# kungyao/vae-play

Hardware: AMD Instinct MI355X
Metric: images/sec (train step, 128x128 VAE) (higher is better)
Workload: dtype bf16x3; 1 GPU; networks VAE 128x128x3 latent=128 train step (fwd+BCE/KL+bwd+allreduce+Adam), 32 images/GPU, global batch 32; parallelism=dp1, per_gpu_batch=32, global_batch=32, graph=False, precision=bf16x3

## Files before the change

### vae_play_amd/csrc/conv16.hip

```cpp
#define VP_PCFG_LIBRARY 1
#define VP_IGEMM16_M16_ON 1
#include "conv16_impl.h"

namespace vp {

__global__ void split_kernel(const float* __restrict__ x, u16_t* __restrict__ out, size_t n, int fmt, float scale) {
  const size_t n4 = n / 4;
  for (size_t i = (size_t)blockIdx.x * blockDim.x + threadIdx.x; i < n4; i += (size_t)gridDim.x * blockDim.x) {
    const vp_f32x4 v = *reinterpret_cast<const vp_f32x4*>(x + i * 4);
    store_split4(out, n, i * 4, v[0] * scale, v[1] * scale, v[2] * scale, v[3] * scale, fmt);
  }
  if (blockIdx.x == 0 && threadIdx.x < (n & 3)) {
    const size_t i = n4 * 4 + threadIdx.x;
    u16_t h, l;
    split_f32(x[i] * scale, h, l, fmt);
    out[i] = h;
    out[n + i] = l;
  }
}

__global__ void split_pad_kernel(const float* __restrict__ x, u16_t* __restrict__ out, size_t npix, int C, int Cpad) {
  const size_t n = npix * (size_t)Cpad, n4 = n / 4;
  for (size_t i = (size_t)blockIdx.x * blockDim.x + threadIdx.x; i < n4; i += (size_t)gridDim.x * blockDim.x) {
    const size_t e = i * 4, pix = e / Cpad;
    const int c = (int)(e - pix * Cpad);
    const float* src = x + pix * (size_t)C;
    float v[4];
#pragma unroll
    for (int j = 0; j < 4; ++j) v[j] = c + j < C ? src[c + j] : 0.f;
    store_split4(out, n, e, v[0], v[1], v[2], v[3]);
  }
}

template <int MODE, bool SPLIT>
__device__ __forceinline__ void pack_tile(float (*tile)[kTaps + 1], const float* __restrict__ w, void* __restrict__ outv, int Cs,
                                          int Cb, int CsP, int nt, int fixed, int j0, int fmt) {
  const size_t n = (size_t)(MODE == 1 ? CsP : Cs) * Cb * nt;
  const int lim = (MODE == 0 ? Cb : Cs) - j0, lim_out = (MODE == 0 ? Cb : CsP) - j0;
  for (int idx = threadIdx.x; idx < 64 * nt; idx += 256) {
    const int j = idx / nt, t = idx - j * nt;
    if (j < lim) tile[j][t] = w[MODE == 0 ? ((size_t)fixed * Cb + j0 + j) * nt + t : ((size_t)(j0 + j) * Cb + fixed) * nt + t];
  }
  __syncthreads();
  const int inner = MODE == 0 ? Cb : CsP;
  for (int idx = threadIdx.x; idx < 64 * nt; idx += 256) {
    const int t = idx >> 6, j = idx & 63;
    if (j < lim_out) {
      const size_t o = ((size_t)fixed * nt + t) * inner + j0 + j;
      const float v = j < lim ? tile[j][t] : 0.f;
      if constexpr (SPLIT) {
        u16_t h, l;
        split_f32(v, h, l, fmt);
        ((u16_t*)outv)[o] = h;
        ((u16_t*)outv)[n + o] = l;
      } else {
        ((float*)outv)[o] = v;
      }
    }
  }
}

template <int MODE, bool SPLIT>
__global__ void __launch_bounds__(256) pack_w5_tiled_kernel(const float* __restrict__ w, void* __restrict__ outv, int Cs, int Cb,
                                                            int CsP, int nt, int fmt = SPLIT_BF16) {
  __shared__ float tile[64][kTaps + 1];
  pack_tile<MODE, SPLIT>(tile, w, outv, Cs, Cb, CsP, nt, blockIdx.x, blockIdx.y * 64, fmt);
}

template <bool SPLIT>
static int pack_w5_launch(const float* w, void* p0, void* p1, int Cs, int Cb, hipStream_t s, const char* what, int CsP = 0,
                          int nt = kTaps) {
  if (CsP < Cs) CsP = Cs;
  if (p0) hipLaunchKernelGGL((pack_w5_tiled_kernel<0, SPLIT>), dim3(Cs, (Cb + 63) / 64), dim3(256), 0, s, w, p0, Cs, Cb, Cs, nt);
  if (p1) hipLaunchKernelGGL((pack_w5_tiled_kernel<1, SPLIT>), dim3(Cb, (CsP + 63) / 64), dim3(256), 0, s, w, p1, Cs, Cb, CsP, nt);
  return check_launch(what);
}

constexpr int kMaxPackJobs = 32;
struct PackJob { const float* w; void* out; int Cs, Cb, CsP, mode, split, tile_begin; };
struct PackTable { PackJob j[kMaxPackJobs]; int n; };

__global__ void __launch_bounds__(256) pack_w5_batch_kernel(const PackTable tab) {
  __shared__ float tile[64][kTaps + 1];
  int ji = 0;
  for (int k = 1; k < tab.n; ++k)
    if ((int)blockIdx.x >= tab.j[k].tile_begin) ji = k;
  const PackJob& jb = tab.j[ji];
  const int tl = blockIdx.x - jb.tile_begin;
  const int ntile = ((jb.mode == 0 ? jb.Cb : jb.CsP) + 63) / 64;
  const int fixed = tl / ntile, j0 = (tl - fixed * ntile) * 64;
  if (jb.mode == 0) {
    const int fmt = jb.split == 2 ? SPLIT_F16 : SPLIT_BF16;
    if (jb.split) pack_tile<0, true>(tile, jb.w, jb.out, jb.Cs, jb.Cb, jb.CsP, kTaps, fixed, j0, fmt);
    else pack_tile<0, false>(tile, jb.w, jb.out, jb.Cs, jb.Cb, jb.CsP, kTaps, fixed, j0, fmt);
  } else {
    const int fmt = jb.split == 2 ? SPLIT_F16 : SPLIT_BF16;
    if (jb.split) pack_tile<1, true>(tile, jb.w, jb.out, jb.Cs, jb.Cb, jb.CsP, kTaps, fixed, j0, fmt);
    else pack_tile<1, false>(tile, jb.w, jb.out, jb.Cs, jb.Cb, jb.CsP, kTaps, fixed, j0, fmt);
  }
}

int pack_w5_f32_launch(const float* w, float* p0, float* p1, int Cs, int Cb, hipStream_t s, int nt) {
  return pack_w5_launch<false>(w, p0, p1, Cs, Cb, s, "vp_pack_w_f32", 0, nt);
}


static inline int im2col5_gw(int C) { return C == 3 ? 16 : (C == 1 ? 8 : 0); }
static inline int im2col5_kc(int C) { const int g = im2col5_gw(C); return g ? ((5 * g + 31) / 32) * 32 : 0; }

template <int C>
__global__ void __launch_bounds__(256) im2col5s2_split_kernel(const float* __restrict__ x, u16_t* __restrict__ out, int B, int Hb, int Wb,
                                                              int Hs, int Ws, int nchw, int fmt) {
  constexpr int GW = C == 3 ? 16 : 8, KC = ((5 * GW + 31) / 32) * 32, G = KC / 8;
  const size_t npix = (size_t)B * Hs * Ws, n = npix * KC;
  const int row = blockIdx.x, b = row / Hs, hs = row - b * Hs;
  for (int i = threadIdx.x; i < Ws * G; i += blockDim.x) {
    const int ws = i / G, c0 = (i - ws * G) * 8;
    float v[8];
#pragma unroll
    for (int j = 0; j < 8; ++j) {
      const int col = c0 + j, r = col / GW, rem = col - r * GW;
      const int q = rem / C, cin = rem - q * C;
      const int h = 2 * hs - 2 + r, w_ = 2 * ws - 2 + q;
      const bool ok = r < 5 && q < 5 && h >= 0 && h < Hb && w_ >= 0 && w_ < Wb;
      v[j] = ok ? (nchw ? x[(((size_t)b * C + cin) * Hb + h) * Wb + w_] : x[(((size_t)b * Hb + h) * Wb + w_) * C + cin]) : 0.f;
    }
    const size_t o = ((size_t)row * Ws + ws) * KC + c0;
    store_split4(out, n, o, v[0], v[1], v[2], v[3], fmt);
    store_split4(out, n, o + 4, v[4], v[5], v[6], v[7], fmt);
  }
}

template <int C>
__global__ void __launch_bounds__(256) im2col5s2_f32_kernel(const float* __restrict__ x, float* __restrict__ out, int B, int Hb, int Wb,
                                                            int Hs, int Ws, int nchw) {
  constexpr int GW = C == 3 ? 16 : 8, KC = ((5 * GW + 31) / 32) * 32, G = KC / 4;
  const int row = blockIdx.x, b = row / Hs, hs = row - b * Hs;
  for (int i = threadIdx.x; i < Ws * G; i += blockDim.x) {
    const int ws = i / G, c0 = (i - ws * G) * 4;
    vp_f32x4 v;
#pragma unroll
    for (int j = 0; j < 4; ++j) {
      const int col = c0 + j, r = col / GW, rem = col - r * GW;
      const int q = rem / C, cin = rem - q * C;
      const int h = 2 * hs - 2 + r, w_ = 2 * ws - 2 + q;
      const bool ok = r < 5 && q < 5 && h >= 0 && h < Hb && w_ >= 0 && w_ < Wb;
      v[j] = ok ? (nchw ? x[(((size_t)b * C + cin) * Hb + h) * Wb + w_] : x[(((size_t)b * Hb + h) * Wb + w_) * C + cin]) : 0.f;
    }
    *reinterpret_cast<vp_f32x4*>(out + ((size_t)row * Ws + ws) * KC + c0) = v;
  }
}

__global__ void pack_w_im2col5_f32_kernel(const float* __restrict__ w, float* __restrict__ out, int Cout, int C, int GW, int KC) {
  const size_t n = (size_t)Cout * KC;
  for (size_t i = (size_t)blockIdx.x * blockDim.x + threadIdx.x; i < n; i += (size_t)gridDim.x * blockDim.x) {
    const int co = (int)(i / KC), col = (int)(i - (size_t)co * KC);
    const int r = col / GW, rem = col - r * GW, q = rem / C, cin = rem - q * C;
    out[i] = (r < 5 && q < 5) ? w[(((size_t)co * C + cin) * 5 + r) * 5 + q] : 0.f;
  }
}

__global__ void pack_w_im2col5_split_kernel(const float* __restrict__ w, u16_t* __restrict__ out, int Cout, int C, int GW, int KC,
                                            int fmt) {
  const size_t n = (size_t)Cout * KC;
  for (size_t i = (size_t)blockIdx.x * blockDim.x + threadIdx.x; i < n; i += (size_t)gridDim.x * blockDim.x) {
    const int co = (int)(i / KC), col = (int)(i - (size_t)co * KC);
    const int r = col / GW, rem = col - r * GW, q = rem / C, cin = rem - q * C;
    const float v = (r < 5 && q < 5) ? w[(((size_t)co * C + cin) * 5 + r) * 5 + q] : 0.f;
    u16_t h, l;
    split_f32(v, h, l, fmt);
    out[i] = h;
    out[n + i] = l;
  }
}

__global__ void unpack_dw_im2col5_kernel(const float* __restrict__ dwc, float* __restrict__ dw, int Cout, int C, int GW, int KC) {
  const size_t n = (size_t)Cout * C * 25;
  for (size_t i = (size_t)blockIdx.x * blockDim.x + threadIdx.x; i < n; i += (size_t)gridDim.x * blockDim.x) {
    const int q = (int)(i % 5), r = (int)((i / 5) % 5), cin = (int)((i / 25) % C), co = (int)(i / ((size_t)25 * C));
    dw[i] = dwc[(size_t)co * KC + r * GW + q * C + cin];
  }
}

__global__ void __launch_bounds__(256) bn_stats_slab_final_kernel(const float* __restrict__ slab, int G, int tiles_m, int BM, long M, long R,
                                                                  int C, float eps, float momentum, float* __restrict__ mean,
                                                                  float* __restrict__ rstd, float* __restrict__ rm, float* __restrict__ rv) {
  __shared__ double shs[4], shq[4];
  const int c = blockIdx.x;
  const float* pv = slab + ((size_t)0 * C + c) * G;
  const float* sv = slab + ((size_t)1 * C + c) * G;
  const float* qv = slab + ((size_t)2 * C + c) * G;
  const double P = (double)pv[0];
  double S = 0.0, Q = 0.0;
  for (int g = threadIdx.x; g < G; g += 256) {
    const int tile = g % tiles_m;
    const long left = M - (long)tile * BM;
    const double n = (double)(left < BM ? left : BM);
    const double d = (double)pv[g] - P, s = (double)sv[g], q = (double)qv[g];
    S += s + n * d;
    Q += q + 2.0 * d * s + n * d * d;
  }
  S = wave_sum_d(S);
  Q = wave_sum_d(Q);
  if ((threadIdx.x & 63) == 0) { shs[threadIdx.x >> 6] = S; shq[threadIdx.x >> 6] = Q; }
  __syncthreads();
  if (threadIdx.x != 0) return;
  S = (shs[0] + shs[1]) + (shs[2] + shs[3]);
  Q = (shq[0] + shq[1]) + (shq[2] + shq[3]);
  const double ms = S / (double)R;
  double var = Q / (double)R - ms * ms;
  if (var < 0.0) var = 0.0;
  const double m = P + ms;
  mean[c] = (float)m;
  rstd[c] = (float)(1.0 / sqrt(var + (double)eps));
  if (rm) rm[c] = (1.f - momentum) * rm[c] + momentum * (float)m;
  if (rv) {
    const double unb = R > 1 ? var * (double)R / (double)(R - 1) : var;
    rv[c] = (1.f - momentum) * rv[c] + momentum * (float)unb;
  }
}

int stats_finish(const ConvPlan& pl, const StatOut& o, hipStream_t stream, const char* what) {
  hipLaunchKernelGGL(bn_stats_slab_final_kernel, dim3((unsigned)pl.N), dim3(256), 0, stream, (const float*)o.ws, pl.stat_tiles_m * pl.gz,
                     pl.stat_tiles_m, pl.bm, pl.M, pl.stat_R, (int)pl.N, o.eps, o.momentum, o.mean, o.rstd, o.running_mean, o.running_var);
  return check_launch(what);
}

}

using namespace vp;
extern "C" {

static bool split_fmt_ok(int fmt, float scale) { return (fmt == SPLIT_BF16 || fmt == SPLIT_F16) && scale > 0.f; }

int vp_split_fmt_f32(const float* x, void* out_split, size_t n, int fmt, float scale, vp_stream stream) {
  VP_REQUIRE(x && out_split && n > 0, "vp_split_fmt_f32: bad arguments");
  VP_REQUIRE(split_fmt_ok(fmt, scale), "vp_split_fmt_f32: format 0 (bf16 pair) or 1 (fp16 pair), scale > 0");
  hipLaunchKernelGGL(split_kernel, dim3(grid_for(n / 4 + 1, 256)), dim3(256), 0, (hipStream_t)stream, x, (u16_t*)out_split, n, fmt, scale);
  return check_launch("vp_split_fmt_f32");
}

int vp_split_f32(const float* x, void* out_split, size_t n, vp_stream stream) {
  return vp_split_fmt_f32(x, out_split, n, SPLIT_BF16, 1.f, stream);
}

int vp_split_pad_f32(const float* x, void* out_split, size_t npix, int C, int Cpad, vp_stream stream) {
  VP_REQUIRE(x && out_split && npix > 0 && C > 0 && Cpad >= C && Cpad % 8 == 0, "vp_split_pad_f32: Cpad must be a multiple of 8 and >= C");
  hipLaunchKernelGGL(split_pad_kernel, dim3(grid_for(npix * (size_t)Cpad / 4 + 1, 256)), dim3(256), 0, (hipStream_t)stream, x,
                     (u16_t*)out_split, npix, C, Cpad);
  return check_launch("vp_split_pad_f32");
}

int vp_pack_w5_split(const float* w_ref, void* p0_split, void* p1_split, int Csmall, int Cbig, vp_stream stream) {
  VP_REQUIRE(w_ref && (p0_split || p1_split) && Csmall > 0 && Cbig > 0, "vp_pack_w5_split: bad arguments");
  VP_REQUIRE(Csmall <= 65535 && Cbig <= 65535, "vp_pack_w5_split: channel count too large");
  return pack_w5_launch<true>(w_ref, p0_split, p1_split, Csmall, Cbig, (hipStream_t)stream, "vp_pack_w5_split");
}

int vp_pack_w5_batch(const vp_pack_job* jobs, int njobs, vp_stream stream) {
  VP_REQUIRE(jobs && njobs > 0, "vp_pack_w5_batch: bad arguments");
  PackTable tab;
  tab.n = 0;
  int tiles = 0;
  for (int i = 0; i < njobs; ++i) {
    const vp_pack_job& q = jobs[i];
    VP_REQUIRE(q.w && (q.p0 || q.p1) && q.Csmall > 0 && q.Cbig > 0, "vp_pack_w5_batch: job %d: bad arguments", i);
    VP_REQUIRE(q.Csmall <= 65535 && q.Cbig <= 65535, "vp_pack_w5_batch: job %d: channel count too large", i);
    const int CsP = q.Csmall_pad > q.Csmall ? q.Csmall_pad : q.Csmall;
    VP_REQUIRE(CsP == q.Csmall || (q.split && CsP % 8 == 0), "vp_pack_w5_batch: job %d: padding needs split planes and a multiple of 8", i);
    for (int mode = 0; mode < 2; ++mode) {
      void* out = mode == 0 ? q.p0 : q.p1;
      if (!out) continue;
      VP_REQUIRE(tab.n < kMaxPackJobs, "vp_pack_w5_batch: more than %d layouts in one batch", kMaxPackJobs);
      PackJob& j = tab.j[tab.n++];
      j.w = q.w; j.out = out; j.Cs = q.Csmall; j.Cb = q.Cbig; j.CsP = mode == 1 ? CsP : q.Csmall; j.mode = mode;
      j.split = q.split == 2 ? 2 : (q.split ? 1 : 0); j.tile_begin = tiles;
      tiles += mode == 0 ? q.Csmall * ((q.Cbig + 63) / 64) : q.Cbig * ((CsP + 63) / 64);
    }
  }
  hipLaunchKernelGGL(pack_w5_batch_kernel, dim3((unsigned)tiles), dim3(256), 0, (hipStream_t)stream, tab);
  return check_launch("vp_pack_w5_batch");
}

int vp_pack_w5_p1_split_padded(const float* w_ref, void* p1_split, int Csmall, int Cbig, int Csmall_pad, vp_stream stream) {
  VP_REQUIRE(w_ref && p1_split && Csmall > 0 && Cbig > 0 && Csmall_pad >= Csmall && Csmall_pad % 8 == 0,
             "vp_pack_w5_p1_split_padded: bad arguments");
  return pack_w5_launch<true>(w_ref, nullptr, p1_split, Csmall, Cbig, (hipStream_t)stream, "vp_pack_w5_p1_split_padded", Csmall_pad);
}

int vp_conv5_gather_bf16x3(const void* big_split, const void* w_p0_split, const float* bias, float* small_out, int B, int Hs,
                           int Ws, int Cbig, int Csmall, int stride, int act, vp_stream stream) {
  return gather16<0>("vp_conv5_gather_bf16x3", big_split, w_p0_split, bias, small_out, B, Hs, Ws, Hs * stride, Ws * stride, Cbig, Csmall, 5, stride, act, stream);
}

int vp_conv_gather_bf16x3(const void* big_split, const void* w_p0_split, const float* bias, float* small_out, int B, int Hs, int Ws,
                          int Hb, int Wb, int Cbig, int Csmall, int ks, int stride, int act, vp_stream stream) {
  return gather16<0>("vp_conv_gather_bf16x3", big_split, w_p0_split, bias, small_out, B, Hs, Ws, Hb, Wb, Cbig, Csmall, ks, stride, act, stream);
}

int vp_conv5_scatter_bf16x3(const void* small_split, const void* w_p1_split, float* big_out, int B, int Hs, int Ws, int Csmall,
                            int Cbig, int stride, vp_stream stream) {
  return scatter16<0>("vp_conv5_scatter_bf16x3", small_split, w_p1_split, big_out, B, Hs, Ws, Hs * stride, Ws * stride, Csmall, Cbig, 5, stride, stream);
}

int vp_conv_scatter_bf16x3(const void* small_split, const void* w_p1_split, float* big_out, int B, int Hs, int Ws, int Hb, int Wb,
                           int Csmall, int Cbig, int ks, int stride, vp_stream stream) {
  return scatter16<0>("vp_conv_scatter_bf16x3", small_split, w_p1_split, big_out, B, Hs, Ws, Hb, Wb, Csmall, Cbig, ks, stride, stream);
}

int vp_conv_scatter_bias_bf16x3(const void* small_split, const void* w_p1_split, const float* bias, float* big_out, int B, int Hs, int Ws,
                                int Hb, int Wb, int Csmall, int Cbig, int ks, int stride, vp_stream stream) {
  return scatter16<0>("vp_conv_scatter_bias_bf16x3", small_split, w_p1_split, big_out, B, Hs, Ws, Hb, Wb, Csmall, Cbig, ks, stride, stream, 1.f, bias);
}

int vp_pack_w_split(const float* w_ref, void* p0_split, void* p1_split, int Csmall, int Cbig, int ks, vp_stream stream) {
  VP_REQUIRE(w_ref && (p0_split || p1_split) && Csmall > 0 && Cbig > 0, "vp_pack_w_split: bad arguments");
  VP_REQUIRE(ks == 1 || ks == 3 || ks == 4 || ks == 5, "vp_pack_w_split: kernel size must be 1, 3, 4 or 5");
  VP_REQUIRE(Csmall <= 65535 && Cbig <= 65535, "vp_pack_w_split: channel count too large");
  return pack_w5_launch<true>(w_ref, p0_split, p1_split, Csmall, Cbig, (hipStream_t)stream, "vp_pack_w_split", 0, ks * ks);
}

size_t vp_conv5_wgrad_bf16x3_workspace_bytes(int B, int Hs, int Ws, int Cbig, int Csmall, int stride) {
  return vp_conv_wgrad_bf16x3_workspace_bytes(B, Hs, Ws, Hs * stride, Ws * stride, Cbig, Csmall, 5, stride);
}

size_t vp_conv_wgrad_bf16x3_workspace_bytes(int B, int Hs, int Ws, int Hb, int Wb, int Cbig, int Csmall, int ks, int stride) {
  const ConvGeom g = make_geom(B, Hs, Ws, Csmall, Cbig, stride, ks, Hb, Wb);
  return plan_wgrad(g, BF16X3, 0, SIZE_MAX, true, plan_switches()).query_floats * sizeof(float);
}

int vp_conv5_wgrad_bf16x3(const void* big_split, const void* small_split, float* dw_ref, int B, int Hs, int Ws, int Cbig,
                          int Csmall, int stride, void* ws, size_t ws_bytes, vp_stream stream) {
  return wgrad16<0>("vp_conv5_wgrad_bf16x3", big_split, small_split, dw_ref, B, Hs, Ws, Hs * stride, Ws * stride, Cbig, Csmall, 5, stride, ws, ws_bytes, stream);
}

int vp_conv5_wgrad_bf16x3_cus(const void* big_split, const void* small_split, float* dw_ref, int B, int Hs, int Ws, int Cbig,
                              int Csmall, int stride, int max_cus, void* ws, size_t ws_bytes, vp_stream stream) {
  return wgrad16<0>("vp_conv5_wgrad_bf16x3_cus", big_split, small_split, dw_ref, B, Hs, Ws, Hs * stride, Ws * stride, Cbig, Csmall, 5, stride, ws, ws_bytes, stream, 1.f, max_cus);
}

int vp_conv_wgrad_bf16x3(const void* big_split, const void* small_split, float* dw_ref, int B, int Hs, int Ws, int Hb, int Wb, int Cbig,
                         int Csmall, int ks, int stride, void* ws, size_t ws_bytes, vp_stream stream) {
  return wgrad16<0>("vp_conv_wgrad_bf16x3", big_split, small_split, dw_ref, B, Hs, Ws, Hb, Wb, Cbig, Csmall, ks, stride, ws, ws_bytes, stream);
}

size_t vp_conv5_stats_workspace_bytes(int family, int B, int Hs, int Ws, int Cbig, int Csmall, int stride) {
  return plan_stats(family, BF16X3, B, Hs, Ws, Cbig, Csmall, stride, true, plan_switches()).stat_floats * sizeof(float);
}

int vp_conv5_gather_stats_bf16x3(const void* big_split, const void* w_p0_split, float* small_out, int B, int Hs, int Ws, int Cbig,
                                 int Csmall, int stride, float eps, float momentum, float* mean, float* rstd, float* running_mean,
                                 float* running_var, void* ws, size_t ws_bytes, vp_stream stream) {
  return conv5_stats("vp_conv5_gather_stats_bf16x3", "vp_conv5_stats_workspace_bytes", conv_gather<ProbF16, FORMS_ALL, TILES_ALL>, 0, BF16X3, true,
                     big_split, w_p0_split, small_out, B, Hs, Ws, Cbig, Csmall, stride,
                     {eps, momentum, mean, rstd, running_mean, running_var, ws, ws_bytes}, stream);
}

int vp_conv5_scatter_stats_bf16x3(const void* small_split, const void* w_p1_split, float* big_out, int B, int Hs, int Ws, int Csmall,
                                  int Cbig, int stride, float eps, float momentum, float* mean, float* rstd, float* running_mean,
                                  float* running_var, void* ws, size_t ws_bytes, vp_stream stream) {
// ... 73 lines not shown
```

### vae_play_amd/csrc/gemm.hip

```cpp
#include "common.h"
#include "igemm.h"

namespace vp {

__global__ void gemm_reduce_kernel(const float* __restrict__ slab, float* __restrict__ C, const float* __restrict__ bias,
                                   int M, int N, int ldc, int nsplit) {
  const size_t per = (size_t)M * N;
  for (size_t i = (size_t)blockIdx.x * blockDim.x + threadIdx.x; i < per; i += (size_t)gridDim.x * blockDim.x) {
    const int n = (int)(i % N);
    const size_t m = i / N;
    float s = bias ? bias[n] : 0.f;
    for (int sp = 0; sp < nsplit; ++sp) s += slab[(size_t)sp * per + i];
    C[m * ldc + n] = s;
  }
}

__global__ void __launch_bounds__(256) gemm_reduce_deep_kernel(const float* __restrict__ slab, float* __restrict__ C,
                                                               const float* __restrict__ bias, int M, int N, int ldc, int nsplit) {
  __shared__ float red[4][64];
  const size_t per = (size_t)M * N;
  const size_t i = (size_t)blockIdx.x * 64 + (threadIdx.x & 63);
  const int sl = threadIdx.x >> 6;
  float s0 = 0.f, s1 = 0.f, s2 = 0.f, s3 = 0.f;
  if (i < per) {
// ... 3 lines not shown
      s1 += slab[(size_t)(sp + 4) * per + i];
      s2 += slab[(size_t)(sp + 8) * per + i];
      s3 += slab[(size_t)(sp + 12) * per + i];
    }
    for (; sp < nsplit; sp += 4) s0 += slab[(size_t)sp * per + i];
  }
  red[sl][threadIdx.x & 63] = (s0 + s1) + (s2 + s3);
  __syncthreads();
  if (sl == 0 && i < per) {
    const int n = (int)(i % N);
    const size_t m = i / N;
    const float v = (red[0][threadIdx.x] + red[1][threadIdx.x]) + (red[2][threadIdx.x] + red[3][threadIdx.x]);
    C[m * ldc + n] = v + (bias ? bias[n] : 0.f);
  }
}

__global__ void colsum_partial_kernel(const float* __restrict__ x, float* __restrict__ partial, int R, int C, int rows_per_chunk) {
  const int chunk = blockIdx.x;
  const int r0 = chunk * rows_per_chunk;
  const int r1 = min(R, r0 + rows_per_chunk);
  for (int c = threadIdx.y; c < C; c += blockDim.y) {
    float s = 0.f;
    for (int r = r0 + threadIdx.x; r < r1; r += blockDim.x) s += x[(size_t)r * C + c];
    s = wave_sum(s);
    if (threadIdx.x == 0) partial[(size_t)chunk * C + c] = s;
  }
}

__global__ void __launch_bounds__(256) colsum_rows4_kernel(const float* __restrict__ x, float* __restrict__ partial, int R, int C,
                                                           int rows_per_chunk) {
  __shared__ vp_f32x4 sh[256];
  const int q = C / 4, rpp = 256 / q;
  const int rl = threadIdx.x / q, c4 = threadIdx.x - rl * q;
  const int r0 = blockIdx.x * rows_per_chunk, r1 = min(R, r0 + rows_per_chunk);
  vp_f32x4 s = {0.f, 0.f, 0.f, 0.f};
  if (rl < rpp) {
    int r = r0 + rl;
    for (; r + 3 * rpp < r1; r += 4 * rpp) {
      const vp_f32x4 a = *reinterpret_cast<const vp_f32x4*>(x + (size_t)r * C + 4 * c4);
      const vp_f32x4 b = *reinterpret_cast<const vp_f32x4*>(x + (size_t)(r + rpp) * C + 4 * c4);
      const vp_f32x4 c = *reinterpret_cast<const vp_f32x4*>(x + (size_t)(r + 2 * rpp) * C + 4 * c4);
      const vp_f32x4 d = *reinterpret_cast<const vp_f32x4*>(x + (size_t)(r + 3 * rpp) * C + 4 * c4);
#pragma unroll
      for (int j = 0; j < 4; ++j) s[j] += (a[j] + b[j]) + (c[j] + d[j]);
    }
    for (; r < r1; r += rpp) {
      const vp_f32x4 a = *reinterpret_cast<const vp_f32x4*>(x + (size_t)r * C + 4 * c4);
#pragma unroll
      for (int j = 0; j < 4; ++j) s[j] += a[j];
    }
  }
  sh[threadIdx.x] = s;
  __syncthreads();
  if (threadIdx.x < q) {
    vp_f32x4 t = sh[threadIdx.x];
    for (int k = 1; k < rpp; ++k) {
      const vp_f32x4 u = sh[k * q + threadIdx.x];
#pragma unroll
      for (int j = 0; j < 4; ++j) t[j] += u[j];
    }
    *reinterpret_cast<vp_f32x4*>(partial + (size_t)blockIdx.x * C + 4 * threadIdx.x) = t;
  }
}

__global__ void __launch_bounds__(256) colsum_wide_kernel(const float* __restrict__ x, float* __restrict__ partial, int R, int C,
                                                          int rows_per_chunk) {
  const int c = blockIdx.x * 256 + threadIdx.x;
  if (c >= C) return;
  const int r0 = blockIdx.y * rows_per_chunk, r1 = min(R, r0 + rows_per_chunk);
  float s = 0.f;
  for (int r = r0; r < r1; ++r) s += x[(size_t)r * C + c];
  partial[(size_t)blockIdx.y * C + c] = s;
}

__global__ void colsum_final_kernel(const float* __restrict__ partial, float* __restrict__ out, int C, int nchunk) {
  const int c = blockIdx.x;
  double s = 0.0;
  for (int k = threadIdx.x; k < nchunk; k += 64) s += (double)partial[(size_t)k * C + c];
  s = wave_sum_d(s);
  if (threadIdx.x == 0) out[c] = (float)s;
}

constexpr int SK_KT = 64;

template <int TM>
__global__ void __launch_bounds__(256) skinny_mk_kernel(const float* __restrict__ A, long sam, const float* __restrict__ Bm, long sbn,
                                                        float* __restrict__ C, int ldc, const float* __restrict__ bias, int M, int N,
                                                        int K, int nsplit, int kps) {
  __shared__ __attribute__((aligned(16))) float xs[2][32 * TM][SK_KT + 4];
  const int tid = threadIdx.x, lane = tid & 63, wave = tid >> 6;
  const int li = lane & 31, lh = lane >> 5;
  const int n = blockIdx.x * 128 + wave * 32 + li;
  const float* wrow = Bm + (size_t)(n < N ? n : 0) * sbn;
  const int k_begin = blockIdx.y * kps;
  const int k_end = min(K, k_begin + kps);
  const int nk = (k_end - k_begin) / SK_KT;
  const int xrow = tid >> 3, xc = tid & 7;
  const float* arow[TM];
  bool xok[TM];
#pragma unroll
  for (int b = 0; b < TM; ++b) {
    xok[b] = xrow + 32 * b < M;
    arow[b] = A + (size_t)(xok[b] ? xrow + 32 * b : 0) * sam;
  }
  vp_f32x4 xr[TM][2], w[8], wn[8];
  f32x16 acc[TM];
#pragma unroll
  for (int b = 0; b < TM; ++b)
#pragma unroll
    for (int r = 0; r < 16; ++r) acc[b][r] = 0.f;
  auto load_tile = [&](int kb) {
#pragma unroll
    for (int b = 0; b < TM; ++b) {
      xr[b][0] = xok[b] ? ld4(arow[b] + kb + xc * 4) : zero4();
      xr[b][1] = xok[b] ? ld4(arow[b] + kb + 32 + xc * 4) : zero4();
    }
#pragma unroll
    for (int i = 0; i < 8; ++i) wn[i] = ld4(wrow + kb + lh * 32 + i * 4);
  };
  auto write_x = [&](int buf) {
#pragma unroll
    for (int b = 0; b < TM; ++b) {
      *reinterpret_cast<vp_f32x4*>(&xs[buf][xrow + 32 * b][xc * 4]) = xr[b][0];
      *reinterpret_cast<vp_f32x4*>(&xs[buf][xrow + 32 * b][32 + xc * 4]) = xr[b][1];
    }
  };
  if (nk > 0) {
    load_tile(k_begin);
    write_x(0);
    __syncthreads();
  }
  for (int t = 0; t < nk; ++t) {
    const bool more = t + 1 < nk;
#pragma unroll
    for (int i = 0; i < 8; ++i) w[i] = wn[i];
    if (more) load_tile(k_begin + (t + 1) * SK_KT);
    const int cur = t & 1;
#pragma unroll
    for (int i = 0; i < 8; ++i) {
      vp_f32x4 x4[TM];
#pragma unroll
      for (int b = 0; b < TM; ++b) x4[b] = *reinterpret_cast<const vp_f32x4*>(&xs[cur][li + 32 * b][lh * 32 + i * 4]);
#pragma unroll
      for (int j = 0; j < 4; ++j)
#pragma unroll
        for (int b = 0; b < TM; ++b) acc[b] = __builtin_amdgcn_mfma_f32_32x32x2f32(x4[b][j], w[i][j], acc[b], 0, 0, 0);
    }
    if (more) write_x(cur ^ 1);
    __syncthreads();
  }
  if (n >= N) return;
#pragma unroll
  for (int b = 0; b < TM; ++b)
#pragma unroll
    for (int r = 0; r < 16; ++r) {
      const int m = 32 * b + (r & 3) + 8 * (r >> 2) + 4 * lh;
      if (m >= M) continue;
      if (nsplit == 1) C[(size_t)m * ldc + n] = acc[b][r] + (bias ? bias[n] : 0.f);
      else C[((size_t)blockIdx.y * M + m) * N + n] = acc[b][r];
    }
}

template <int TM>
__global__ void __launch_bounds__(256) skinny_kn_kernel(const float* __restrict__ A, long sam, const float* __restrict__ Bm, long sbk,
                                                        float* __restrict__ C, int ldc, const float* __restrict__ bias, int M, int N,
                                                        int K, int nsplit, int kps) {
// ... 10 lines not shown
    aok[b] = li + 32 * b < M;
    arow[b] = A + (size_t)(aok[b] ? li + 32 * b : 0) * sam;
  }
  const int k_begin = blockIdx.y * kps;
  const int k_end = min(K, k_begin + kps);
  const int nk = (k_end - k_begin) / SK_KT;
  f32x16 acc[TM][4];
#pragma unroll
  for (int b = 0; b < TM; ++b)
#pragma unroll
    for (int c = 0; c < 4; ++c)
#pragma unroll
      for (int r = 0; r < 16; ++r) acc[b][c][r] = 0.f;
  vp_f32x4 w[8], wn[8], a[TM][2], an[TM][2];
  auto load_half = [&](int kb) {
#pragma unroll
    for (int q = 0; q < 2; ++q) {
#pragma unroll
      for (int b = 0; b < TM; ++b) an[b][q] = aok[b] ? ld4(arow[b] + kb + q * 8 + lh * 4) : zero4();
#pragma unroll
      for (int j = 0; j < 4; ++j) wn[q * 4 + j] = ld4(wcol + (size_t)(kb + q * 8 + lh * 4 + j) * sbk);
    }
  };
  const int nh = nk > wave ? ((nk - wave + 3) / 4) * 4 : 0;
  auto kb_of = [&](int h) { return k_begin + (wave + 4 * (h >> 2)) * SK_KT + (h & 3) * 16; };
  if (nh > 0) load_half(kb_of(0));
  for (int h = 0; h < nh; ++h) {
#pragma unroll
    for (int i = 0; i < 8; ++i) w[i] = wn[i];
#pragma unroll
    for (int b = 0; b < TM; ++b) { a[b][0] = an[b][0]; a[b][1] = an[b][1]; }
    if (h + 1 < nh) load_half(kb_of(h + 1));
#pragma unroll
    for (int q = 0; q < 2; ++q)
#pragma unroll
      for (int j = 0; j < 4; ++j)
#pragma unroll
        for (int c = 0; c < 4; ++c)
#pragma unroll
          for (int b = 0; b < TM; ++b)
            acc[b][c] = __builtin_amdgcn_mfma_f32_32x32x2f32(a[b][q][j], w[q * 4 + j][c], acc[b][c], 0, 0, 0);
  }
#pragma unroll
  for (int b = 0; b < TM; ++b) {
    __syncthreads();
    if (wave >= 2) {
#pragma unroll
      for (int c = 0; c < 4; ++c)
#pragma unroll
        for (int r = 0; r < 16; ++r) red[wave - 2][c * 16 + r][lane] = acc[b][c][r];
    }
    __syncthreads();
    if (wave < 2) {
#pragma unroll
      for (int c = 0; c < 4; ++c)
#pragma unroll
        for (int r = 0; r < 16; ++r) acc[b][c][r] += red[wave][c * 16 + r][lane];
    }
    __syncthreads();
    if (wave == 1) {
#pragma unroll
      for (int c = 0; c < 4; ++c)
#pragma unroll
        for (int r = 0; r < 16; ++r) red[0][c * 16 + r][lane] = acc[b][c][r];
    }
    __syncthreads();
    if (wave == 0 && nok) {
#pragma unroll
      for (int r = 0; r < 16; ++r) {
        const int m = 32 * b + (r & 3) + 8 * (r >> 2) + 4 * lh;
        if (m >= M) continue;
        vp_f32x4 v;
#pragma unroll
        for (int c = 0; c < 4; ++c) v[c] = acc[b][c][r] + red[0][c * 16 + r][lane];
        if (nsplit == 1) {
          if (bias) { v[0] += bias[n0]; v[1] += bias[n0 + 1]; v[2] += bias[n0 + 2]; v[3] += bias[n0 + 3]; }
          *reinterpret_cast<vp_f32x4*>(C + (size_t)m * ldc + n0) = v;
        } else {
          *reinterpret_cast<vp_f32x4*>(C + ((size_t)blockIdx.y * M + m) * N + n0) = v;
        }
      }
    }
  }
}

inline int skinny_nsplit(int mode, long M, long N, long K) {
  if (mode > 1 || M > 64 || N < 128 || K % SK_KT) return 0;
  const long colblocks = (N + 127) / 128;
  const long unit = mode == 0 ? 256 : 4 * SK_KT;
  long blocks = 512;
  long want = (blocks + colblocks - 1) / colblocks;
  long maxs = K / unit;
  if (maxs < 1) maxs = 1;
  long s = want < maxs ? want : maxs;
  if (s > 128) s = 128;
  return (int)s;
}
inline int skinny_kps(long K, int ns) {
  const long per = (K + ns - 1) / ns;
  return (int)(((per + SK_KT - 1) / SK_KT) * SK_KT);
}

__global__ void __launch_bounds__(256) colsum_small_kernel(const float* __restrict__ x, float* __restrict__ out, int R, int C) {
  const int c = blockIdx.x * 256 + threadIdx.x;
  if (c >= C) return;
  float s = 0.f;
  for (int r = 0; r < R; ++r) s += x[(size_t)r * C + c];
  out[c] = s;
}

inline int colsum_chunks(int R) {
  int n = (R + 511) / 512;
  if (n > 1024) n = 1024;
  if (n < 1) n = 1;
  return n;
}

}

using namespace vp;

extern "C" {

size_t vp_gemm_workspace_bytes(int M, int N, int K) {
  int ns = gemm_nsplit(M, N, K);
  for (int mode = 0; mode < 2; ++mode) {
    const int s0 = skinny_nsplit(mode, M, N, K);
    if (s0) { const int kps = skinny_kps(K, s0); const int eff = (K + kps - 1) / kps; if (eff > ns) ns = eff; }
  }
  return ns > 1 ? (size_t)ns * M * N * sizeof(float) : 0;
}

int vp_gemm_f32(const float* A, long sam, long sak, const float* B, long sbn, long sbk, float* C, int ldc,
                const float* bias, int M, int N, int K, int mode, void* ws, size_t ws_bytes, vp_stream stream) {
  VP_REQUIRE(A && B && C, "vp_gemm_f32: null pointer");
  VP_REQUIRE(M > 0 && N > 0 && K > 0 && ldc >= N, "vp_gemm_f32: bad shape M=%d N=%d K=%d ldc=%d", M, N, K, ldc);
  VP_REQUIRE(mode >= 0 && mode <= 2, "vp_gemm_f32: mode must be 0|1|2");
  int ns = gemm_nsplit(M, N, K);
  const auto al16 = [](const void* q) { return ((uintptr_t)q & 15) == 0; };
  int sk = skinny_nsplit(mode, M, N, K);
  if (sk && mode == 0 && !(sak == 1 && sbk == 1 && sam % 4 == 0 && sbn % 4 == 0 && al16(A) && al16(B))) sk = 0;
  if (sk && mode == 1 && !(sak == 1 && sbn == 1 && sam % 4 == 0 && sbk % 4 == 0 && N % 4 == 0 && ldc % 4 == 0 && al16(A) && al16(B) && al16(C))) sk = 0;
  if (sk) {
    const int kps = skinny_kps(K, sk);
    ns = (K + kps - 1) / kps;
    float* dst = C;
    if (ns > 1) {
      if (!ws || ws_bytes < (size_t)ns * M * N * sizeof(float)) return fail(VP_ERR_WORKSPACE, "vp_gemm_f32: workspace too small");
      dst = (float*)ws;
    }
    hipStream_t s = (hipStream_t)stream;
    const dim3 grid((unsigned)((N + 127) / 128), (unsigned)ns);
    if (mode == 0 && M <= 32) hipLaunchKernelGGL(skinny_mk_kernel<1>, grid, dim3(256), 0, s, A, sam, B, sbn, dst, ldc, bias, M, N, K, ns, kps);
    else if (mode == 0) hipLaunchKernelGGL(skinny_mk_kernel<2>, grid, dim3(256), 0, s, A, sam, B, sbn, dst, ldc, bias, M, N, K, ns, kps);
    else if (M <= 32) hipLaunchKernelGGL(skinny_kn_kernel<1>, grid, dim3(256), 0, s, A, sam, B, sbk, dst, ldc, bias, M, N, K, ns, kps);
    else hipLaunchKernelGGL(skinny_kn_kernel<2>, grid, dim3(256), 0, s, A, sam, B, sbk, dst, ldc, bias, M, N, K, ns, kps);
    int rc = check_launch("vp_gemm_f32(skinny)");
    if (rc || ns == 1) return rc;
    if (ns >= 16 && (size_t)M * N <= 65536)
      hipLaunchKernelGGL(gemm_reduce_deep_kernel, dim3((unsigned)(((size_t)M * N + 63) / 64)), dim3(256), 0, s, (const float*)ws, C, bias, M, N, ldc, ns);
    else
      hipLaunchKernelGGL(gemm_reduce_kernel, dim3(grid_for((size_t)M * N, 256)), dim3(256), 0, s, (const float*)ws, C, bias, M, N, ldc, ns);
    return check_launch("vp_gemm_f32(reduce)");
  }
  float* dst = C;
  if (ns > 1) {
    const size_t need = (size_t)ns * M * N * sizeof(float);
    if (!ws || ws_bytes < need) return fail(VP_ERR_WORKSPACE, "vp_gemm_f32: workspace %zu < %zu", ws_bytes, need);
    dst = (float*)ws;
  }
  hipStream_t s = (hipStream_t)stream;
  if (mode == 0) {
    auto p = make_probG<false, false>(A, sam, sak, B, sbn, sbk, dst, ldc, bias, M, N, K, ns);
    launch_igemm(p, M, N, ns, s);
  } else if (mode == 1) {
    auto p = make_probG<false, true>(A, sam, sak, B, sbn, sbk, dst, ldc, bias, M, N, K, ns);
    launch_igemm(p, M, N, ns, s);
  } else {
    auto p = make_probG<true, true>(A, sam, sak, B, sbn, sbk, dst, ldc, bias, M, N, K, ns);
    launch_igemm(p, M, N, ns, s);
  }
  int rc = check_launch("vp_gemm_f32(main)");
  if (rc || ns == 1) return rc;
  if (ns >= 16 && (size_t)M * N <= 65536)
    hipLaunchKernelGGL(gemm_reduce_deep_kernel, dim3((unsigned)(((size_t)M * N + 63) / 64)), dim3(256), 0, s, (const float*)ws, C, bias, M, N, ldc, ns);
  else
    hipLaunchKernelGGL(gemm_reduce_kernel, dim3(grid_for((size_t)M * N, 256)), dim3(256), 0, s, (const float*)ws, C, bias, M, N, ldc, ns);
  return check_launch("vp_gemm_f32(reduce)");
}

size_t vp_colsum_workspace_bytes(int R, int C) { return (size_t)colsum_chunks(R) * C * sizeof(float); }

int vp_colsum_f32(const float* x, float* out, int R, int C, void* ws, size_t ws_bytes, vp_stream stream) {
  VP_REQUIRE(x && out && ws && R > 0 && C > 0, "vp_colsum_f32: bad arguments");
  const bool small_on = true;
  if (R <= 64 && small_on) {
    hipLaunchKernelGGL(colsum_small_kernel, dim3((C + 255) / 256), dim3(256), 0, (hipStream_t)stream, x, out, R, C);
    return check_launch("vp_colsum_f32(small)");
  }
  const int nchunk = colsum_chunks(R);
  if (ws_bytes < (size_t)nchunk * C * sizeof(float)) return fail(VP_ERR_WORKSPACE, "vp_colsum_f32: workspace too small");
  const int rpc = (R + nchunk - 1) / nchunk;
  hipStream_t s = (hipStream_t)stream;
  if (C >= 64)
    hipLaunchKernelGGL(colsum_wide_kernel, dim3((C + 255) / 256, nchunk), dim3(256), 0, s, x, (float*)ws, R, C, rpc);
  else if (C % 4 == 0 && C >= 8 && ((uintptr_t)x & 15) == 0)
    hipLaunchKernelGGL(colsum_rows4_kernel, dim3(nchunk), dim3(256), 0, s, x, (float*)ws, R, C, rpc);
  else
    hipLaunchKernelGGL(colsum_partial_kernel, dim3(nchunk), dim3(64, 4), 0, s, x, (float*)ws, R, C, rpc);
  int rc = check_launch("vp_colsum_f32(partial)");
  if (rc) return rc;
  hipLaunchKernelGGL(colsum_final_kernel, dim3(C), dim3(64), 0, s, (const float*)ws, out, C, nchunk);
  return check_launch("vp_colsum_f32(final)");
}
}
```

Measured before the change: 9192 images/sec.

## Pack both weight layouts from one shared-memory tile in batched pack kernel

Result: no change. 9238 images/sec (median of 5 runs) (+0.5%).

```diff
diff --git a/vae_play_amd/csrc/conv16.hip b/vae_play_amd/csrc/conv16.hip
--- a/vae_play_amd/csrc/conv16.hip
+++ b/vae_play_amd/csrc/conv16.hip
@@ -1,6 +1,11 @@
 #define VP_PCFG_LIBRARY 1
 #define VP_IGEMM16_M16_ON 1
 #include "conv16_impl.h"
+
+#ifndef VP_PACK_BOTH_CS
+#define VP_PACK_BOTH_CS 16
+#define VP_PACK_BOTH_CB 32
+#endif
 
 namespace vp {
 
@@ -77,24 +82,86 @@
 }
 
 constexpr int kMaxPackJobs = 32;
-struct PackJob { const float* w; void* out; int Cs, Cb, CsP, mode, split, tile_begin; };
+struct PackJob { const float* w; void* out; void* out1; int Cs, Cb, CsP, mode, split, tile_begin; };
 struct PackTable { PackJob j[kMaxPackJobs]; int n; };
 
+constexpr int kBothCs = VP_PACK_BOTH_CS, kBothCb = VP_PACK_BOTH_CB;
+constexpr int kBothLds = kBothCs * kBothCb * kTaps;
+static_assert(kBothCs % 8 == 0 && kBothCb % 8 == 0 && kBothLds >= 64 * (kTaps + 1), "tile of pack_tile_both");
+
+__device__ __forceinline__ void store_split8(u16_t* plane, size_t n, size_t o, const float (&v)[8], int fmt) {
+  union { u16_t s[8]; vp_f32x4 q; } h, l;
+#pragma unroll
+  for (int k = 0; k < 8; ++k) split_f32(v[k], h.s[k], l.s[k], fmt);
+  *reinterpret_cast<vp_f32x4*>(plane + o) = h.q;
+  *reinterpret_cast<vp_f32x4*>(plane + n + o) = l.q;
+}
+
+__device__ __forceinline__ void pack_tile_both(float* __restrict__ sm, const float* __restrict__ w, u16_t* __restrict__ p0,
+                                               u16_t* __restrict__ p1, int Cs, int Cb, int CsP, int cs0, int cb0, int fmt) {
+  constexpr int SCS = kBothCb * kTaps;
+  const int ncs = max(0, min(kBothCs, Cs - cs0)), ncb = min(kBothCb, Cb - cb0);
+  const int run4 = ncb * kTaps / 4;
+  const int nld = ncs * run4;
+  for (int base = threadIdx.x; base < nld; base += 4 * 256) {
+    vp_f32x4 r[4];
+#pragma unroll
+    for (int u = 0; u < 4; ++u) {
+      const int idx = min(base + u * 256, nld - 1), cs = idx / run4, v = idx - cs * run4;
+      r[u] = ld4(w + ((size_t)(cs0 + cs) * Cb + cb0) * kTaps + v * 4);
+    }
+#pragma unroll
+    for (int u = 0; u < 4; ++u) {
+      const int idx = base + u * 256, cs = idx / run4, v = idx - cs * run4;
+      if (idx < nld) *reinterpret_cast<vp_f32x4*>(sm + cs * SCS + v * 4) = r[u];
+    }
+  }
+  __syncthreads();
+  {
+    const size_t n = (size_t)Cs * Cb * kTaps;
+    const int G = ncb / 8;
+    for (int idx = threadIdx.x; idx < ncs * kTaps * G; idx += 256) {
+      const int g = idx % G, ct = idx / G, cs = ct / kTaps, t = ct - cs * kTaps;
+      float v[8];
+#pragma unroll
+      for (int k = 0; k < 8; ++k) v[k] = sm[cs * SCS + (g * 8 + k) * kTaps + t];
+      store_split8(p0, n, ((size_t)(cs0 + cs) * kTaps + t) * Cb + cb0 + g * 8, v, fmt);
+    }
+  }
+  {
+    const size_t n = (size_t)CsP * Cb * kTaps;
+    const int H = (min(kBothCs, CsP - cs0) + 7) / 8;
+    for (int idx = threadIdx.x; idx < ncb * kTaps * H; idx += 256) {
+      const int h = idx % H, q = idx / H;
+      float v[8];
+#pragma unroll
+      for (int k = 0; k < 8; ++k) v[k] = h * 8 + k < ncs ? sm[(h * 8 + k) * SCS + q] : 0.f;
+      store_split8(p1, n, ((size_t)cb0 * kTaps + q) * CsP + cs0 + h * 8, v, fmt);
+    }
+  }
+}
+
 __global__ void __launch_bounds__(256) pack_w5_batch_kernel(const PackTable tab) {
-  __shared__ float tile[64][kTaps + 1];
+  __shared__ __attribute__((aligned(16))) float sm[kBothLds];
   int ji = 0;
   for (int k = 1; k < tab.n; ++k)
     if ((int)blockIdx.x >= tab.j[k].tile_begin) ji = k;
   const PackJob& jb = tab.j[ji];
   const int tl = blockIdx.x - jb.tile_begin;
+  const int fmt = jb.split == 2 ? SPLIT_F16 : SPLIT_BF16;
+  if (jb.mode == 2) {
+    const int ntile = (jb.Cb + kBothCb - 1) / kBothCb;
+    const int ts = tl / ntile;
+    pack_tile_both(sm, jb.w, (u16_t*)jb.out, (u16_t*)jb.out1, jb.Cs, jb.Cb, jb.CsP, ts * kBothCs, (tl - ts * ntile) * kBothCb, fmt);
+    return;
+  }
+  float (*tile)[kTaps + 1] = reinterpret_cast<float (*)[kTaps + 1]>(sm);
   const int ntile = ((jb.mode == 0 ? jb.Cb : jb.CsP) + 63) / 64;
   const int fixed = tl / ntile, j0 = (tl - fixed * ntile) * 64;
   if (jb.mode == 0) {
-    const int fmt = jb.split == 2 ? SPLIT_F16 : SPLIT_BF16;
     if (jb.split) pack_tile<0, true>(tile, jb.w, jb.out, jb.Cs, jb.Cb, jb.CsP, kTaps, fixed, j0, fmt);
     else pack_tile<0, false>(tile, jb.w, jb.out, jb.Cs, jb.Cb, jb.CsP, kTaps, fixed, j0, fmt);
   } else {
-    const int fmt = jb.split == 2 ? SPLIT_F16 : SPLIT_BF16;
     if (jb.split) pack_tile<1, true>(tile, jb.w, jb.out, jb.Cs, jb.Cb, jb.CsP, kTaps, fixed, j0, fmt);
     else pack_tile<1, false>(tile, jb.w, jb.out, jb.Cs, jb.Cb, jb.CsP, kTaps, fixed, j0, fmt);
   }
@@ -261,21 +328,27 @@
   VP_REQUIRE(jobs && njobs > 0, "vp_pack_w5_batch: bad arguments");
   PackTable tab;
   tab.n = 0;
-  int tiles = 0;
+  int tiles = 0, layouts = 0;
   for (int i = 0; i < njobs; ++i) {
     const vp_pack_job& q = jobs[i];
     VP_REQUIRE(q.w && (q.p0 || q.p1) && q.Csmall > 0 && q.Cbig > 0, "vp_pack_w5_batch: job %d: bad arguments", i);
     VP_REQUIRE(q.Csmall <= 65535 && q.Cbig <= 65535, "vp_pack_w5_batch: job %d: channel count too large", i);
     const int CsP = q.Csmall_pad > q.Csmall ? q.Csmall_pad : q.Csmall;
     VP_REQUIRE(CsP == q.Csmall || (q.split && CsP % 8 == 0), "vp_pack_w5_batch: job %d: padding needs split planes and a multiple of 8", i);
+    const int split = q.split == 2 ? 2 : (q.split ? 1 : 0);
+    const bool both = q.p0 && q.p1 && split && q.Cbig % 8 == 0 && CsP % 8 == 0 && aligned16((const char*)q.w, (const char*)q.p0, (const char*)q.p1);
     for (int mode = 0; mode < 2; ++mode) {
       void* out = mode == 0 ? q.p0 : q.p1;
       if (!out) continue;
-      VP_REQUIRE(tab.n < kMaxPackJobs, "vp_pack_w5_batch: more than %d layouts in one batch", kMaxPackJobs);
+      VP_REQUIRE(layouts < kMaxPackJobs, "vp_pack_w5_batch: more than %d layouts in one batch", kMaxPackJobs);
+      ++layouts;
+      if (both && mode == 1) continue;
       PackJob& j = tab.j[tab.n++];
-      j.w = q.w; j.out = out; j.Cs = q.Csmall; j.Cb = q.Cbig; j.CsP = mode == 1 ? CsP : q.Csmall; j.mode = mode;
-      j.split = q.split == 2 ? 2 : (q.split ? 1 : 0); j.tile_begin = tiles;
-      tiles += mode == 0 ? q.Csmall * ((q.Cbig + 63) / 64) : q.Cbig * ((CsP + 63) / 64);
+      j.w = q.w; j.out = out; j.out1 = both ? q.p1 : nullptr; j.Cs = q.Csmall; j.Cb = q.Cbig;
+      j.CsP = (mode == 1 || both) ? CsP : q.Csmall; j.mode = both ? 2 : mode;
+      j.split = split; j.tile_begin = tiles;
+      if (both) tiles += ((CsP + kBothCs - 1) / kBothCs) * ((q.Cbig + kBothCb - 1) / kBothCb);
+      else tiles += mode == 0 ? q.Csmall * ((q.Cbig + 63) / 64) : q.Cbig * ((CsP + 63) / 64);
     }
   }
   hipLaunchKernelGGL(pack_w5_batch_kernel, dim3((unsigned)tiles), dim3(256), 0, (hipStream_t)stream, tab);
```

## Add register-ring prefetch stream kernels for skinny dense GEMMs

Applied to the files above, without the earlier changes.

Measured after the change: 9244 images/sec before, 9319 images/sec after, median of 6. Within noise of the previous version (+0.8%).

```diff
diff --git a/vae_play_amd/csrc/gemm.hip b/vae_play_amd/csrc/gemm.hip
--- a/vae_play_amd/csrc/gemm.hip
+++ b/vae_play_amd/csrc/gemm.hip
@@ -109,6 +109,7 @@
 }
 
 constexpr int SK_KT = 64;
+
 
 template <int TM>
 __global__ void __launch_bounds__(256) skinny_mk_kernel(const float* __restrict__ A, long sam, const float* __restrict__ Bm, long sbn,
@@ -285,6 +286,219 @@
       }
     }
   }
+}
+
+template <int D, int OFF, class Issue, class Pre, class Post>
+__device__ __forceinline__ void ring_groups(int n, Issue issue, Pre pre, Post post) {
+#pragma unroll
+  for (int d = OFF; d < D; ++d) issue(d - OFF, d);
+  int t = -OFF;
+  if (n + OFF > D) {
+#pragma unroll
+    for (int d = 0; d < D; ++d) {
+      if (d >= OFF) pre(t + d, d);
+      issue(t + d + D, d);
+      if (d >= OFF) post(t + d, d);
+    }
+    for (t += D; t + D < n; t += D) {
+#pragma unroll
+      for (int d = 0; d < D; ++d) { pre(t + d, d); issue(t + d + D, d); post(t + d, d); }
+    }
+#pragma unroll
+    for (int d = 0; d < D; ++d) { pre(t + d, d); post(t + d, d); }
+  } else {
+#pragma unroll
+    for (int d = OFF; d < D; ++d) { pre(t + d, d); post(t + d, d); }
+  }
+}
+template <int D, class Issue, class Pre, class Post>
+__device__ __forceinline__ void ring(int n, Issue issue, Pre pre, Post post) {
+  static_assert(D >= 1 && D <= 3, "ring depth");
+  if (n <= 0) return;
+  const int off = (D - n % D) % D;
+  if (off == 0) ring_groups<D, 0>(n, issue, pre, post);
+  else if (off == 1) ring_groups<D, (D > 1 ? 1 : 0)>(n, issue, pre, post);
+  else ring_groups<D, (D > 2 ? 2 : 0)>(n, issue, pre, post);
+}
+
+__device__ __forceinline__ vp_f32x4 ldw4_nt(const float* p) { return __builtin_nontemporal_load(reinterpret_cast<const vp_f32x4*>(p)); }
+
+constexpr int ST_P = SK_KT + 4;
+
+template <int TM, int D>
+__global__ void __launch_bounds__(256, 2) stream_mk_kernel(const float* __restrict__ A, long sam, const float* __restrict__ Bm, long sbn,
+                                                        float* __restrict__ C, int ldc, const float* __restrict__ bias, int M, int N,
+                                                        int K, int nsplit, int kps) {
+  constexpr int NB = TM == 1 ? 2 : 1;
+  __shared__ __attribute__((aligned(16))) float xs[NB][32 * TM][ST_P];
+  __shared__ __attribute__((aligned(16))) float wsh[4][32][ST_P];
+  const int tid = threadIdx.x, lane = tid & 63, wave = tid >> 6;
+  const int li = lane & 31, lh = lane >> 5;
+  const int lq = lane >> 4, lc = lane & 15;
+  const int nbase = blockIdx.x * 128 + wave * 32;
+  const int n = nbase + li;
+  const int k_begin = blockIdx.y * kps;
+  const int k_end = min(K, k_begin + kps);
+  const int nk = (k_end - k_begin) / SK_KT;
+  const float* wp[8];
+#pragma unroll
+  for (int i = 0; i < 8; ++i) {
+    const int r = nbase + 4 * i + lq;
+    wp[i] = Bm + (size_t)(r < N ? r : 0) * sbn + k_begin + lc * 4;
+  }
+  const int xrow = tid >> 3, xc = tid & 7;
+  const float* arow[TM];
+  bool xok[TM];
+#pragma unroll
+  for (int b = 0; b < TM; ++b) {
+    xok[b] = xrow + 32 * b < M;
+    arow[b] = A + (size_t)(xok[b] ? xrow + 32 * b : 0) * sam + k_begin + xc * 4;
+  }
+  vp_f32x4 wr[D][8], xr[D][TM][2];
+  f32x16 acc[TM];
+#pragma unroll
+  for (int b = 0; b < TM; ++b)
+#pragma unroll
+    for (int r = 0; r < 16; ++r) acc[b][r] = 0.f;
+  auto issue = [&](int t, int d) {
+#pragma unroll
+    for (int b = 0; b < TM; ++b) {
+      xr[d][b][0] = ld4(arow[b] + t * SK_KT);
+      xr[d][b][1] = ld4(arow[b] + t * SK_KT + 32);
+    }
+#pragma unroll
+    for (int i = 0; i < 8; ++i) wr[d][i] = ldw4_nt(wp[i] + t * SK_KT);
+  };
+  auto stage = [&](int t, int d) {
+    const int buf = NB == 2 ? (t & 1) : 0;
+    if (NB == 1) __syncthreads();
+#pragma unroll
+    for (int b = 0; b < TM; ++b) {
+      *reinterpret_cast<vp_f32x4*>(&xs[buf][xrow + 32 * b][xc * 4]) = xok[b] ? xr[d][b][0] : zero4();
+      *reinterpret_cast<vp_f32x4*>(&xs[buf][xrow + 32 * b][32 + xc * 4]) = xok[b] ? xr[d][b][1] : zero4();
+    }
+#pragma unroll
+    for (int i = 0; i < 8; ++i) *reinterpret_cast<vp_f32x4*>(&wsh[wave][4 * i + lq][lc * 4]) = wr[d][i];
+  };
+  auto compute = [&](int t, int) {
+    const int buf = NB == 2 ? (t & 1) : 0;
+    __syncthreads();
+#pragma unroll
+    for (int i = 0; i < 8; ++i) {
+      const vp_f32x4 w4 = *reinterpret_cast<const vp_f32x4*>(&wsh[wave][li][lh * 32 + i * 4]);
+      vp_f32x4 x4[TM];
+#pragma unroll
+      for (int b = 0; b < TM; ++b) x4[b] = *reinterpret_cast<const vp_f32x4*>(&xs[buf][li + 32 * b][lh * 32 + i * 4]);
+#pragma unroll
+      for (int j = 0; j < 4; ++j)
+#pragma unroll
+        for (int b = 0; b < TM; ++b) acc[b] = __builtin_amdgcn_mfma_f32_32x32x2f32(x4[b][j], w4[j], acc[b], 0, 0, 0);
+    }
+  };
+  ring<D>(nk, issue, stage, compute);
+  if (n >= N) return;
+#pragma unroll
+  for (int b = 0; b < TM; ++b)
+#pragma unroll
+    for (int r = 0; r < 16; ++r) {
+      const int m = 32 * b + (r & 3) + 8 * (r >> 2) + 4 * lh;
+      if (m >= M) continue;
+      if (nsplit == 1) C[(size_t)m * ldc + n] = acc[b][r] + (bias ? bias[n] : 0.f);
+      else C[((size_t)blockIdx.y * M + m) * N + n] = acc[b][r];
+    }
+}
+
+template <int TM, int D>
+__global__ void __launch_bounds__(256, 2) stream_kn_kernel(const float* __restrict__ A, long sam, const float* __restrict__ Bm, long sbk,
+                                                        float* __restrict__ C, int ldc, const float* __restrict__ bias, int M, int N,
+                                                        int K, int nsplit, int kps) {
+  __shared__ __attribute__((aligned(16))) float red[4][3][16][64];
+  const int tid = threadIdx.x, lane = tid & 63, wave = tid >> 6;
+  const int li = lane & 31, lh = lane >> 5;
+  const int n0 = blockIdx.x * 128 + 4 * li;
+  const bool nok = n0 < N;
+  const float* wcol = Bm + (nok ? n0 : 0);
+  const float* arow[TM];
+#pragma unroll
+  for (int b = 0; b < TM; ++b)
+    arow[b] = A + (size_t)(li + 32 * b < M ? li + 32 * b : 0) * sam;
+  const int k_begin = blockIdx.y * kps;
+  const int k_end = min(K, k_begin + kps);
+  const int nk = (k_end - k_begin) / SK_KT;
+  f32x16 acc[TM][4];
+#pragma unroll
+  for (int b = 0; b < TM; ++b)
+#pragma unroll
+    for (int c = 0; c < 4; ++c)
+#pragma unroll
+      for (int r = 0; r < 16; ++r) acc[b][c][r] = 0.f;
+  vp_f32x4 w[D][8], a[D][TM][2];
+  const int nh = nk > wave ? ((nk - wave + 3) / 4) * 4 : 0;
+  auto kb_of = [&](int h) { return k_begin + (wave + 4 * (h >> 2)) * SK_KT + (h & 3) * 16; };
+  auto issue = [&](int h, int d) {
+    const int kb = kb_of(h);
+#pragma unroll
+    for (int q = 0; q < 2; ++q) {
+#pragma unroll
+      for (int b = 0; b < TM; ++b) a[d][b][q] = ld4(arow[b] + kb + q * 8 + lh * 4);
+#pragma unroll
+      for (int j = 0; j < 4; ++j) w[d][q * 4 + j] = ldw4_nt(wcol + (size_t)(kb + q * 8 + lh * 4 + j) * sbk);
+    }
+  };
+  auto step = [&](int, int d) {
+#pragma unroll
+    for (int q = 0; q < 2; ++q)
+#pragma unroll
+      for (int j = 0; j < 4; ++j)
+#pragma unroll
+        for (int c = 0; c < 4; ++c)
+#pragma unroll
+          for (int b = 0; b < TM; ++b)
+            acc[b][c] = __builtin_amdgcn_mfma_f32_32x32x2f32(a[d][b][q][j], w[d][q * 4 + j][c], acc[b][c], 0, 0, 0);
+  };
+  ring<D>(nh, issue, step, [](int, int) {});
+#pragma unroll
+  for (int b = 0; b < TM; ++b) {
+    if (b) __syncthreads();
+#pragma unroll
+    for (int g = 0; g < 4; ++g) {
+      if (g == wave) continue;
+      const int slot = wave < g ? wave : wave - 1;
+#pragma unroll
+      for (int c = 0; c < 4; ++c)
+#pragma unroll
+        for (int rr = 0; rr < 4; ++rr) red[g][slot][c * 4 + rr][lane] = acc[b][c][4 * g + rr];
+    }
+    __syncthreads();
+#pragma unroll
+    for (int g = 0; g < 4; ++g) {
+      if (g != wave || !nok) continue;
+#pragma unroll
+      for (int rr = 0; rr < 4; ++rr) {
+        const int m = 32 * b + rr + 8 * g + 4 * lh;
+        if (m >= M) continue;
+        vp_f32x4 v;
+#pragma unroll
+        for (int c = 0; c < 4; ++c) {
+          float p[4];
+#pragma unroll
+          for (int s = 0; s < 4; ++s) p[s] = s == g ? acc[b][c][4 * g + rr] : red[g][s < g ? s : s - 1][c * 4 + rr][lane];
+          v[c] = ((p[0] + p[1]) + p[2]) + p[3];
+        }
+        if (nsplit == 1) {
+          if (bias) { v[0] += bias[n0]; v[1] += bias[n0 + 1]; v[2] += bias[n0 + 2]; v[3] += bias[n0 + 3]; }
+          *reinterpret_cast<vp_f32x4*>(C + (size_t)m * ldc + n0) = v;
+        } else {
+          *reinterpret_cast<vp_f32x4*>(C + ((size_t)blockIdx.y * M + m) * N + n0) = v;
+        }
+      }
+    }
+  }
+}
+
+inline int dense_stream_value() {
+  const char* e = VP_GETENV("VP_DENSE_STREAM");
+  return e ? atoi(e) : 1;
 }
 
 inline int skinny_nsplit(int mode, long M, long N, long K) {
@@ -354,7 +568,15 @@
     }
     hipStream_t s = (hipStream_t)stream;
     const dim3 grid((unsigned)((N + 127) / 128), (unsigned)ns);
-    if (mode == 0 && M <= 32) hipLaunchKernelGGL(skinny_mk_kernel<1>, grid, dim3(256), 0, s, A, sam, B, sbn, dst, ldc, bias, M, N, K, ns, kps);
+    const int dsv = dense_stream_value();
+    if (mode == 0 && dsv != 0) {
+      if (M <= 32) hipLaunchKernelGGL((stream_mk_kernel<1, 3>), grid, dim3(256), 0, s, A, sam, B, sbn, dst, ldc, bias, M, N, K, ns, kps);
+      else hipLaunchKernelGGL((stream_mk_kernel<2, 2>), grid, dim3(256), 0, s, A, sam, B, sbn, dst, ldc, bias, M, N, K, ns, kps);
+    } else if (mode == 1 && dsv == 3) {
+      if (M <= 32) hipLaunchKernelGGL((stream_kn_kernel<1, 3>), grid, dim3(256), 0, s, A, sam, B, sbk, dst, ldc, bias, M, N, K, ns, kps);
+      else hipLaunchKernelGGL((stream_kn_kernel<2, 2>), grid, dim3(256), 0, s, A, sam, B, sbk, dst, ldc, bias, M, N, K, ns, kps);
+    }
+    else if (mode == 0 && M <= 32) hipLaunchKernelGGL(skinny_mk_kernel<1>, grid, dim3(256), 0, s, A, sam, B, sbn, dst, ldc, bias, M, N, K, ns, kps);
     else if (mode == 0) hipLaunchKernelGGL(skinny_mk_kernel<2>, grid, dim3(256), 0, s, A, sam, B, sbn, dst, ldc, bias, M, N, K, ns, kps);
     else if (M <= 32) hipLaunchKernelGGL(skinny_kn_kernel<1>, grid, dim3(256), 0, s, A, sam, B, sbk, dst, ldc, bias, M, N, K, ns, kps);
     else hipLaunchKernelGGL(skinny_kn_kernel<2>, grid, dim3(256), 0, s, A, sam, B, sbk, dst, ldc, bias, M, N, K, ns, kps);
```
